# agis85/multimodal_segmentation

Hardware: AMD Instinct MI355X
Metric: 2D slices/sec DAFNet train step, 256x256x2-modality bs=8/GPU (higher is better)
Workload: dtype f32

## Files before the change

### include/mmseg_hip.h

```cpp
#ifndef MMSEG_HIP_H
#define MMSEG_HIP_H

#ifdef __cplusplus
extern "C" {
#endif

#define MMSEG_ACT_NONE 0
#define MMSEG_ACT_RELU 1
#define MMSEG_ACT_LEAKY 2
#define MMSEG_ACT_TANH 3

int mmseg_conv2d_fwd(const float* x1, const float* x2, const float* w, const float* wt, const float* bias, float* y, float* y2,
                     int B, int H, int W, int C1, int C2, int Ho, int Wo, int Cout, int KH, int KW, int stride,
                     int pad_h, int pad_w, int ups, int transposed, int act, float alpha, int nsplit1, void* stream);
int mmseg_set_conv_precision(int mode);
int mmseg_conv16_mode(int mode);
int mmseg_get_conv_precision(void);
int mmseg_conv2d_fwd_scaled(const float* x1, const float* x2, const float* w, const float* wt, const float* bias, const float* oscale,
                            float* y, int B, int H, int W, int C1, int C2, int Ho, int Wo, int Cout, int KH, int KW, int stride,
                            int pad_h, int pad_w, int ups, int act, float alpha, void* stream);
int mmseg_conv2d_fwd_t(const void* x1, const void* x2, const float* w, const float* wt, const float* bias, void* y, void* y2,
                       int B, int H, int W, int C1, int C2, int Ho, int Wo, int Cout, int KH, int KW, int stride,
                       int pad_h, int pad_w, int ups, int transposed, int act, float alpha, int nsplit1, int io, void* stream);
int mmseg_conv2d_fwd_scaled_t(const void* x1, const void* x2, const float* w, const float* wt, const float* bias, const float* oscale,
// ... 94 lines not shown
int mmseg_cat_words(const void* p0, const void* p1, const void* p2, const void* p3, const void* p4, const void* p5, const void* p6,
                    const void* p7, int n, void* out, long words, void* stream);
int mmseg_gather_rows(const void* src, const long long* idx, void* out, int rows, long words, int src_rows, void* stream);
int mmseg_add_residual(const float* msk, float* out, long M, int C, void* stream);
int mmseg_act_bwd_bias_t(const void* dy, const void* y, void* dx, float* bias_grad, float* ws, long M, int C, int act, float alpha,
                         int accumulate, int h, void* stream);
int mmseg_im2col8_t(const void* x, void* out, int B, int H, int W, int hx, int hy, void* stream);
int mmseg_conv8h_fwd_t(const void* x, const float* w, const float* bias, void* y, int B, int H, int W, int Cout, int act, float alpha,
                       int hx, int hy, void* stream);
int mmseg_in_workspace_floats(int B);
int mmseg_instnorm_spade_fwd(const float* x, const float* gamma, const float* beta, float* y, float* stat, float* ws, int B,
                             long per_sample, float eps, float act_alpha, void* stream);
int mmseg_instnorm_spade_bwd(const float* dy, const float* x, const float* stat, const float* gamma, const float* beta, float* dx,
                             float* dgamma, float* dbeta, float* dxn, float* ws, int B, long per_sample, float eps, float act_alpha,
                             void* stream);
int mmseg_instnorm_spade_fwd_gb(const float* x, const float* gb, float* y, float* stat, float* ws, int B, long per_sample, int C, float eps,
                                float act_alpha, void* stream);
int mmseg_instnorm_spade_bwd_gb(const float* dy, const float* x, const float* stat, const float* gb, float* dx, float* dgb, float* dxn,
                                float* ws, int B, long per_sample, int C, float eps, float act_alpha, void* stream);
int mmseg_instnorm_spade_fwd_gb_t(const float* x, const void* gb, void* y, float* stat, float* ws, int B, long per_sample, int C, float eps,
                                  float act_alpha, int h, int hy, void* stream);
int mmseg_instnorm_spade_bwd_gb_t(const void* dy, const float* x, const float* stat, const void* gb, float* dx, void* dgb, float* dxn,
                                  float* ws, int B, long per_sample, int C, float eps, float act_alpha, int h, int hy, void* stream);
int mmseg_colsum_t(const void* x, float* out, float* ws, long M, int C, int accumulate, int h, void* stream);
int mmseg_concat_cols(const float* a, const float* b, float* out, long M, int Ca, int Cb, void* stream);
int mmseg_split_cols_acc(const float* src, float* da, float* db, long M, int Ca, int Cb, void* stream);


long mmseg_dense_workspace_floats(int R, int K, int N);
int mmseg_dense_fwd(const float* x, const float* w, const float* bias, float* y, float* ws, int R, int K, int N, int act,
                    float alpha, void* stream);
int mmseg_dense_dgrad(const float* dy, const float* w, float* dx, int R, int K, int N, void* stream);
int mmseg_dense_wgrad(const float* x, const float* dy, float* dw, int R, int K, int N, int accumulate, void* stream);

int mmseg_tps_workspace_floats(int B);
int mmseg_tps_warp_fwd(const float* vol, const float* theta, const float* Mb, float* out, float* loc, int B, int H, int W, int C,
                       void* stream);
long mmseg_tps_scatter_workspace_floats(int B, int H, int W, int C);
int mmseg_tps_warp_bwd(const float* vol, const float* loc, const float* Mb, const float* dout, float* dvol, float* dtheta, float* dloc,
                       float* ws, float* acc, int B, int H, int W, int C, void* stream);

int mmseg_affine_gather(const float* data, const int* rows, const float* mat, float* out, int B, int H, int W, int C, int order,
                        void* stream);
long mmseg_augment_workspace_floats(int B, int H, int W, int C);
int mmseg_augment_gather(const float* data, const int* rows, const double* mat, const float* shift, float* out, float* ws, int N,
                         int B, int H, int W, int C, int order, int fill_mode, float cval, void* stream);

int mmseg_segloss_workspace_floats(int B);
int mmseg_segloss_stats_floats(int B);
int mmseg_segloss_coef_floats(int B, int C);
int mmseg_segloss_class_offset(int B);
int mmseg_segloss_stats(const float* pred, const float* target, float* stats, float* ws, int B, long HW, int C, int nm, void* stream);
int mmseg_segloss_finalize(const float* stats, float* loss, float* coef, int B, int C, float n_pix_global, float n_pix_grad,
                           float lambda_bce, void* stream);
int mmseg_segloss_grad(const float* pred, const float* target, const float* coef, float* dpred, int B, long HW, int C, int nm,
                       float scale, int use_bce, void* stream);
int mmseg_segloss_grad_s(const float* pred, const float* target, const float* coef, float* dpred, int B, long HW, int C, int nm,
                         float scale, const float* scale_dev, int use_bce, void* stream);
int mmseg_pairloss_workspace_floats(int B);
int mmseg_pair_dice_fwd(const float* a, const float* b, float* stats, float* out, int ldo, float* ws, int B, long per_sample,
                        void* stream);
int mmseg_pair_dice_bwd(const float* a, const float* b, const float* stats, const float* g, int ldg, float* da, float* db,
                        int accumulate_a, int B, long per_sample, void* stream);
int mmseg_row_mae_fwd(const float* x, const float* y, float* out, float* ws, int B, long per_sample, void* stream);
int mmseg_row_mae_bwd(const float* x, const float* y, const float* g, float* dy, int B, long per_sample, void* stream);
int mmseg_segpb_stats_floats(int B);
int mmseg_segpb_class_offset(int B);
int mmseg_segpb_stats(const float* pred, const float* target, float* stats, float* ws, int B, long HW, int C, int nm, void* stream);
int mmseg_segpb_loss(const float* stats, float* loss, int B, long HW, int C, float lambda_bce, void* stream);
int mmseg_segpb_classgrad(const float* stats, const float* g, float* A, int B, void* stream);
int mmseg_segpb_grad(const float* target, const float* stats, const float* g, const float* A, float* dpred, int B, long HW, int C,
                     int nm, float lambda_bce, void* stream);
int mmseg_rowdot_fwd(const float* w, const float* l, float* out, int B, int J, void* stream);
int mmseg_rowdot_bwd(const float* w, const float* l, const float* g, float* dw, float* dl, int B, int J, void* stream);

int mmseg_diffloss_workspace_floats(void);
int mmseg_diffloss(const float* p, const float* t, float tconst, long n, int mode, float* loss, float* ws, void* stream);
int mmseg_diffloss_grad(const float* p, const float* t, float tconst, long n, int mode, float scale, float* dp, void* stream);
int mmseg_diffloss_grad_s(const float* p, const float* t, float tconst, long n, int mode, float scale, const float* scale_dev, float* dp,
                          void* stream);

int mmseg_adam(float* p, const float* g, float* m, float* v, long n, float lr_t, float b1, float b2, float eps, void* stream);
int mmseg_adam_p(float* p, const float* g, float* m, float* v, long n, const float* lr_t, float b1, float b2, float eps, void* stream);
long mmseg_spectral_workspace_floats(int K, int N);
int mmseg_spectral_fwd(const float* w, const float* u0, float* loss, float* sgn, float* ws, int K, int N, float alpha, void* stream);
int mmseg_spectral_grad(const float* w, const float* sgn, float scale, long n, float* dw, void* stream);
int mmseg_spectral_fwd4(const float* w0, const float* w1, const float* w2, const float* w3, const float* u0, const float* u1,
                        const float* u2, const float* u3, float* loss, float* sgn, float* ws, int n, int K0, int N0, int K1, int N1,
                        int K2, int N2, int K3, int N3, float alpha, void* stream);
int mmseg_spectral_grad4(const float* w0, const float* w1, const float* w2, const float* w3, const float* sgn, float* dw0, float* dw1,
                         float* dw2, float* dw3, int n, long n0, long n1, long n2, long n3, float scale, void* stream);
int mmseg_spectral_grad4_s(const float* w0, const float* w1, const float* w2, const float* w3, const float* sgn, float* dw0, float* dw1,
                           float* dw2, float* dw3, int n, long n0, long n1, long n2, long n3, float scale, const float* scale_dev,
                           void* stream);

int mmseg_unscale_check8(float* g0, float* g1, float* g2, float* g3, float* g4, float* g5, float* g6, float* g7, long n0, long n1,
                         long n2, long n3, long n4, long n5, long n6, long n7, int count, const float* scale, int* st, void* stream);
int mmseg_adam_guarded(float* p, const float* g, float* m, float* v, long n, const float* lr_table, int table_len, const int* st,
                       float b1, float b2, float eps, void* stream);
int mmseg_loss_scale_update(float* scale, int* st, int growth_interval, void* stream);

long mmseg_preprocess_workspace_floats(int S, int RH, int RW);
int mmseg_preprocess_minmax(const float* img, float* ws, int S, int H, int W, int RH, int RW, void* stream);
int mmseg_preprocess_image(const float* img, const float* ws, float* out, int S, int H, int W, int RH, int RW, int OH, int OW, int lo_r,
                           int kept_r, int before_r, int lo_c, int kept_c, int before_c, int C, int ch, void* stream);
int mmseg_preprocess_label(const unsigned char* lab, const int* values, float* out, int S, int H, int W, int RH, int RW, int OH, int OW,
                           int lo_r, int kept_r, int before_r, int lo_c, int kept_c, int before_c, int C, int ch0, int K, void* stream);

int mmseg_restore_label(const float* prob, const int* values, unsigned char* out, int S, int H, int W, int RH, int RW, int OH, int OW,
                        int lo_r, int kept_r, int before_r, int lo_c, int kept_c, int before_c, int C, int K, int order, void* stream);
int mmseg_label_overlap(const unsigned char* pred, const unsigned char* truth, const int* values, int* counts, int S, int n, int K,
                        void* stream);

// ... 35 lines not shown
```

### multimodal_segmentation_amd/csrc/dense.hip

```cpp
#include "common.hpp"

#define DENSE_KSLICES_MAX 1024

static inline int dense_kslices(int K) {
    int ks = (K + 127) / 128;
    if (ks > DENSE_KSLICES_MAX) ks = DENSE_KSLICES_MAX;
    if (ks < 1) ks = 1;
    return ks;
}

template <int RB>
__global__ void dense_fwd_partial_kernel(const float* __restrict__ x, const float* __restrict__ w, float* __restrict__ part,
                                         int R, int K, int N, int kper) {
    __shared__ float red[4][RB][64];
    const int nl = threadIdx.x & 63, kl = threadIdx.x >> 6;
    const int n = blockIdx.x * 64 + nl;
    const int kbeg = blockIdx.y * kper, kend = min(K, kbeg + kper);
    float acc[RB];
#pragma unroll
    for (int b = 0; b < RB; ++b) acc[b] = 0.f;
    if (n < N) {
#pragma unroll 4
        for (int k = kbeg + kl; k < kend; k += 4) {
            const float wv = w[(size_t)k * N + n];
// ... 160 lines not shown
__global__ __launch_bounds__(256) void dense_dgrad_smallk_kernel(const float* __restrict__ dy, const float* __restrict__ w,
                                                                 float* __restrict__ dx, int K, int N) {
    __shared__ float red[17];
    const int b = blockIdx.x;
    float acc[KMAX];
#pragma unroll
    for (int k = 0; k < KMAX; ++k) acc[k] = 0.f;
    for (int n = threadIdx.x; n < N; n += 256) {
        const float d = dy[(size_t)b * N + n];
#pragma unroll
        for (int k = 0; k < KMAX; ++k)
            if (k < K) acc[k] = fmaf(d, w[(size_t)k * N + n], acc[k]);
    }
#pragma unroll
    for (int k = 0; k < KMAX; ++k) {
        if (k < K) {
            const float t = block_sum(acc[k], red);
            if (threadIdx.x == 0) dx[(size_t)b * K + k] = t;
        }
    }
}

__global__ void dense_wgrad_kernel(const float* __restrict__ x, const float* __restrict__ dy, float* __restrict__ dw,
                                   int R, int K, int N, int accumulate) {
    const long total = (long)K * N;
    for (long i = (long)blockIdx.x * blockDim.x + threadIdx.x; i < total; i += (long)gridDim.x * blockDim.x) {
        const int k = i / N, n = i - (long)k * N;
        float a = 0.f;
        for (int b = 0; b < R; ++b) a += x[(size_t)b * K + k] * dy[(size_t)b * N + n];
        dw[i] = accumulate ? dw[i] + a : a;
    }
}

extern "C" {

long mmseg_dense_workspace_floats(int R, int K, int N) {
    const long a = (long)dense_kslices(K) * R * N, b = (long)((K + SMALLN_KPB - 1) / SMALLN_KPB) * R * N;
    return a > b ? a : b;
}

int mmseg_dense_fwd(const float* x, const float* w, const float* bias, float* y, float* ws, int R, int K, int N, int act,
                    float alpha, void* stream) {
    if (R < 1 || R > 32) return (int)hipErrorInvalidValue;
    hipStream_t st = (hipStream_t)stream;
    if (N <= 4 && (R <= 16 || N == 1) && K >= 4096) {
        const int nb = (K + SMALLN_KPB - 1) / SMALLN_KPB;
        if (R > 16) {
            hipLaunchKernelGGL((dense_fwd_smalln_kernel<32, 1>), dim3(nb), dim3(256), 0, st, x, w, ws, R, K, N);
        } else if (R <= 8) {
            if (N == 1) hipLaunchKernelGGL((dense_fwd_smalln_kernel<8, 1>), dim3(nb), dim3(256), 0, st, x, w, ws, R, K, N);
            else hipLaunchKernelGGL((dense_fwd_smalln_kernel<8, 4>), dim3(nb), dim3(256), 0, st, x, w, ws, R, K, N);
        } else {
            if (N == 1) hipLaunchKernelGGL((dense_fwd_smalln_kernel<16, 1>), dim3(nb), dim3(256), 0, st, x, w, ws, R, K, N);
            else hipLaunchKernelGGL((dense_fwd_smalln_kernel<16, 4>), dim3(nb), dim3(256), 0, st, x, w, ws, R, K, N);
        }
        hipLaunchKernelGGL(dense_fwd_final_kernel, dim3((R * N + 63) / 64), dim3(256), 0, st, (const float*)ws, bias, y, R, N, nb, act, alpha);
        return MMSEG_CHECK_LAUNCH();
    }
    const int ks = dense_kslices(K);
    int kper = (K + ks - 1) / ks;
    dim3 grid((N + 63) / 64, ks), block(256);
    if (K % 4 == 0 && (reinterpret_cast<uintptr_t>(x) & 15) == 0) {
        kper = (kper + 3) / 4 * 4;
        if (R <= 8) hipLaunchKernelGGL(dense_fwd_partial_k4_kernel<8>, grid, block, 0, st, x, w, ws, R, K, N, kper);
        else if (R <= 16) hipLaunchKernelGGL(dense_fwd_partial_k4_kernel<16>, grid, block, 0, st, x, w, ws, R, K, N, kper);
        else hipLaunchKernelGGL(dense_fwd_partial_k4_kernel<32>, grid, block, 0, st, x, w, ws, R, K, N, kper);
        hipLaunchKernelGGL(dense_fwd_final_kernel, dim3((R * N + 63) / 64), dim3(256), 0, st, (const float*)ws, bias, y, R, N, ks, act, alpha);
// ... 27 lines not shown
```

### multimodal_segmentation_amd/csrc/loss.hip

```cpp
#include "common.hpp"

#define LOSS_CHUNKS 128
#define SEG_MAXC 8

__global__ void segloss_partial_kernel(const float* __restrict__ pred, const float* __restrict__ target, float* __restrict__ part,
                                       long HW, int C, int nm) {
    __shared__ float red[17];
    const int b = blockIdx.y;
    const long per = (HW + LOSS_CHUNKS - 1) / LOSS_CHUNKS;
    const long p0 = (long)blockIdx.x * per, p1 = min(HW, p0 + per);
    float sI = 0.f, sT = 0.f, sP = 0.f, n[SEG_MAXC], S[SEG_MAXC];
#pragma unroll
    for (int c = 0; c < SEG_MAXC; ++c) { n[c] = 0.f; S[c] = 0.f; }
    for (long px = p0 + threadIdx.x; px < p1; px += blockDim.x) {
        const size_t o = ((size_t)b * HW + px) * C;
#pragma unroll
        for (int c = 0; c < SEG_MAXC; ++c) {
            if (c < C) {
                const float p = pred[o + c], t = target[o + c];
                if (c < nm) { sI += t * p; sT += t; sP += p; }
                n[c] += p;
                S[c] += p * logf(t + 1e-12f);
            }
        }
// ... 108 lines not shown
    if (threadIdx.x == 0) part[blockIdx.x] = a;
}
__global__ void diffloss_final_kernel(const float* __restrict__ part, int nblk, float inv_n, float* __restrict__ loss) {
    __shared__ float red[17];
    float a = 0.f;
    for (int i = threadIdx.x; i < nblk; i += blockDim.x) a += part[i];
    a = block_sum(a, red);
    if (threadIdx.x == 0) loss[0] = a * inv_n;
}
__global__ void diffloss_grad_kernel(const float* __restrict__ p, const float* __restrict__ t, float tconst, long n, int mode,
                                     float scale, float* __restrict__ dp) {
    for (long i = (long)blockIdx.x * blockDim.x + threadIdx.x; i < n; i += (long)gridDim.x * blockDim.x) {
        const float d = p[i] - (t ? t[i] : tconst);
        float g;
        if (mode == 0) g = d > 0.f ? 1.f : (d < 0.f ? -1.f : 0.f);
        else if (mode == 1) g = 2.f * d;
        else g = 1.f;
        dp[i] = g * scale;
    }
}
__global__ void diffloss_grad_s_kernel(const float* __restrict__ p, const float* __restrict__ t, float tconst, long n, int mode,
                                       float scale_host, const float* __restrict__ scale_dev, float* __restrict__ dp) {
    const float scale = scale_host * scale_dev[0];
    for (long i = (long)blockIdx.x * blockDim.x + threadIdx.x; i < n; i += (long)gridDim.x * blockDim.x) {
        const float d = p[i] - (t ? t[i] : tconst);
        float g;
        if (mode == 0) g = d > 0.f ? 1.f : (d < 0.f ? -1.f : 0.f);
        else if (mode == 1) g = 2.f * d;
        else g = 1.f;
        dp[i] = g * scale;
    }
}

static inline int lgrid(long n) {
    long b = (n + 255) / 256;
    if (b > 1024) b = 1024;
    if (b < 1) b = 1;
    return (int)b;
}

extern "C" {

int mmseg_segloss_workspace_floats(int B) { return B * LOSS_CHUNKS * (3 + 2 * SEG_MAXC); }
int mmseg_segloss_stats_floats(int B) { return B * 3 + 2 * SEG_MAXC; }
int mmseg_segloss_coef_floats(int B, int C) { return 2 * B + 2 * C; }
int mmseg_segloss_class_offset(int B) { return 3 * B; }

int mmseg_segloss_stats(const float* pred, const float* target, float* stats, float* ws, int B, long HW, int C, int nm, void* stream) {
    if (C > SEG_MAXC || nm > C || B * 3 > 1024) return (int)hipErrorInvalidValue;
    hipStream_t st = (hipStream_t)stream;
    hipLaunchKernelGGL(segloss_partial_kernel, dim3(LOSS_CHUNKS, B), dim3(256), 0, st, pred, target, ws, HW, C, nm);
    hipLaunchKernelGGL(segloss_stats_final_kernel, dim3(1), dim3(1024), 0, st, (const float*)ws, stats, B);
    return MMSEG_CHECK_LAUNCH();
}
int mmseg_segloss_finalize(const float* stats, float* loss, float* coef, int B, int C, float n_pix_global, float n_pix_grad, float lambda_bce, void* stream) {
    hipLaunchKernelGGL(segloss_finalize_kernel, dim3(1), dim3(64), 0, (hipStream_t)stream, stats, loss, coef, B, C, n_pix_global, n_pix_grad, lambda_bce);
    return MMSEG_CHECK_LAUNCH();
}
int mmseg_segloss_grad(const float* pred, const float* target, const float* coef, float* dpred, int B, long HW, int C, int nm,
                       float scale, int use_bce, void* stream) {
    const long n = (long)B * HW * C;
    hipLaunchKernelGGL(segloss_grad_kernel, dim3(lgrid(n) * 4), dim3(256), 0, (hipStream_t)stream, pred, target, coef, dpred, B, HW, C, nm, scale, use_bce);
    return MMSEG_CHECK_LAUNCH();
}
int mmseg_segloss_grad_s(const float* pred, const float* target, const float* coef, float* dpred, int B, long HW, int C, int nm,
                         float scale, const float* scale_dev, int use_bce, void* stream) {
    if (scale_dev == nullptr) return (int)hipErrorInvalidValue;
    const long n = (long)B * HW * C;
    hipLaunchKernelGGL(segloss_grad_s_kernel, dim3(lgrid(n) * 4), dim3(256), 0, (hipStream_t)stream, pred, target, coef, dpred, B, HW, C,
                       nm, scale, scale_dev, use_bce);
    return MMSEG_CHECK_LAUNCH();
}

int mmseg_diffloss_workspace_floats(void) { return 1024; }
int mmseg_diffloss(const float* p, const float* t, float tconst, long n, int mode, float* loss, float* ws, void* stream) {
    hipStream_t st = (hipStream_t)stream;
    const int nblk = lgrid(n);
    hipLaunchKernelGGL(diffloss_partial_kernel, dim3(nblk), dim3(256), 0, st, p, t, tconst, n, mode, ws);
    hipLaunchKernelGGL(diffloss_final_kernel, dim3(1), dim3(256), 0, st, (const float*)ws, nblk, 1.f / (float)n, loss);
    return MMSEG_CHECK_LAUNCH();
}
int mmseg_diffloss_grad(const float* p, const float* t, float tconst, long n, int mode, float scale, float* dp, void* stream) {
    hipLaunchKernelGGL(diffloss_grad_kernel, dim3(lgrid(n) * 4), dim3(256), 0, (hipStream_t)stream, p, t, tconst, n, mode, scale, dp);
    return MMSEG_CHECK_LAUNCH();
}
int mmseg_diffloss_grad_s(const float* p, const float* t, float tconst, long n, int mode, float scale, const float* scale_dev, float* dp,
                          void* stream) {
    if (scale_dev == nullptr) return (int)hipErrorInvalidValue;
    hipLaunchKernelGGL(diffloss_grad_s_kernel, dim3(lgrid(n) * 4), dim3(256), 0, (hipStream_t)stream, p, t, tconst, n, mode, scale, scale_dev,
                       dp);
    return MMSEG_CHECK_LAUNCH();
}

}
```

### multimodal_segmentation_amd/model_components/decoder.py

```python
import logging

from .. import nn, ops
from ..layers import spade
from ..utils.rng import global_rng

log = logging.getLogger('decoder')


class Decoder(nn.Model):
    def __init__(self, conf, rng):
        super(Decoder, self).__init__('Decoder')
        self.conf = conf
        self.decoder_type = conf.decoder_type
        sc = conf.anatomy_encoder.output_shape[-1]
        if conf.decoder_type == 'film':
            nn.conv_params(self, 'c0', 3, sc, 8)
            for i in range(4):
                nn.conv_params(self, 'f%d_c1' % i, 3, 8, 8)
                nn.conv_params(self, 'f%d_c2' % i, 3, 8, 8)
                nn.dense_params(self, 'f%d_gamma' % i, conf.num_z, 8)
                nn.dense_params(self, 'f%d_beta' % i, conf.num_z, 8)
            last = 8
        elif conf.decoder_type == 'spade':
            last = spade.declare_spade_decoder(self, conf)
        else:
            raise ValueError('Unknown decoder_type value: ' + str(conf.decoder_type))
        nn.conv_params(self, 'out', 1, last, 1, 'glorot_normal')
        self.finalize(rng)
        self.output_shape = (None,) + tuple(conf.input_shape)

    def _film_decoder(self, s, z):
        l = nn.conv(self, 'c0', s, act='leaky', alpha=0.3)
        zs = ops.Shared(z, 8)
        for i in range(4):
            n = 'f%d' % i
            l1 = ops.Shared(nn.conv(self, n + '_c1', l, act='leaky', alpha=0.3), 2)
            l2 = nn.conv(self, n + '_c2', l1.use())
            gamma = nn.dense(self, n + '_gamma', zs.use(), act='leaky', alpha=0.3)
            beta = nn.dense(self, n + '_beta', zs.use(), act='leaky', alpha=0.3)
            l = ops.film(l2, gamma, beta, res=l1.use(), alpha=0.3)
        return l

    def forward(self, s, z, training=False):
        if self.decoder_type == 'film':
            l = self._film_decoder(s, z)
        else:
            l = spade.spade_decoder(self, self.conf, s, z)
        return nn.conv(self, 'out', l, act='tanh')


def build(conf, rng=None):
    model = Decoder(conf, rng or global_rng())
    log.info('Decoder')
    model.summary(print_fn=log.debug)
    return model
```

### multimodal_segmentation_amd/models/trainer.py

```python
import torch

from .. import graphs, nn, ops
from ..parallel import dp


class OutputSpec(object):
    __slots__ = ('name', 'kind', 'weight')

    def __init__(self, name, kind, weight):
        self.name, self.kind, self.weight = name, kind, float(weight)


class Trainer(object):
    def __init__(self, name, graph_fn, output_specs, train_models, optimizer, num_masks=None, regularised=(),
                 all_models=()):
        self.name = name
        self.graph_fn = graph_fn
        self.specs = list(output_specs)
        self.train_models = list(train_models)
        self.optimizer = optimizer
        self.num_masks = num_masks
        self.regularised = list(regularised)
        self.all_models = list(all_models) or self.train_models
        self.device = self.train_models[0].device
        self.last_outputs = None
        self.use_graph = False
        self._graphs = {}
        self.loss_scale = 1.0
        self.scaler = None
        self.precision = None

    @property
    def output_names(self):
        return [s.name for s in self.specs]

    def summary(self, print_fn=print):
        print_fn('Trainer %s: %d outputs, trainable models: %s' % (self.name, len(self.specs),
                                                                   ', '.join(m.name for m in self.train_models)))

    def _loss_and_grad(self, spec, pred, target):
        gs = spec.weight * self.loss_scale
        sd = self.scaler.scale_dev if self.scaler is not None else None
        if spec.kind == 'dice_bce':
            return ops.seg_loss(pred, target, self.num_masks, 0.01, gs, class_sum_hook=dp.class_sum_hook(),
                                n_pix_global=pred.numel() // pred.shape[-1] * dp.world_size(), scale_dev=sd)
        if spec.kind == 'dice':
            return ops.seg_loss(pred, target, self.num_masks, 0.0, gs, scale_dev=sd)
        if spec.kind == 'mse':
            return ops.diff_loss(pred, target, 'mse', gs, scale_dev=sd)
        if spec.kind == 'mae':
            return ops.diff_loss(pred, target, 'mae', gs, scale_dev=sd)
        if spec.kind == 'ypred':
            return ops.diff_loss(pred, 0.0, 'mean', gs, scale_dev=sd)
        raise ValueError(spec.kind)

    def _prep_target(self, t, pred):
        if isinstance(t, (int, float)):
            return float(t)
        t = nn.to_device(t, self.device)
        if t.numel() != pred.numel():
            t = t.reshape(-1, *([1] * (pred.dim() - 1))).expand_as(pred).contiguous()
        return t

    def fit(self, inputs, targets, epochs=1, verbose=0, **graph_kw):
        assert epochs == 1
        inputs = list(inputs) if isinstance(inputs, (list, tuple)) else [inputs]
        targets = list(targets) if isinstance(targets, (list, tuple)) else [targets]
        graph_kw = {k: v for k, v in graph_kw.items() if v is not None}
        with ops.precision_scope(self.precision):
            if self.use_graph and not graph_kw and not dp.enabled() and self.device.type == 'cuda':
                key = graphs.signature(inputs, targets)
                st = self._graphs.get(key)
                if st is None:
                    st = self._graphs[key] = graphs.FitGraph(self)
                return st.run(inputs, targets)
            return self._fit_eager(inputs, targets, graph_kw)

    @staticmethod
    def _total(terms):
        return nn_total(terms)

    def _fit_eager(self, inputs, targets, graph_kw, lr_dev=None):
        ins = [nn.to_device(x, self.device) for x in inputs]
        assert len(targets) == len(self.specs), '%s: %d targets for %d outputs' % (self.name, len(targets), len(self.specs))
        for m in self.train_models:
            m.zero_grad_own()
        tracker = dp.begin(self.train_models, defer=[d for d in self.regularised if d in self.train_models])
        with torch.enable_grad():
            outs = self.graph_fn(ins, **graph_kw)
            assert len(outs) == len(self.specs)
            hist = nn.History()
            grads, terms = [], []
            for spec, pred, tgt in zip(self.specs, outs, targets):
                loss, dpred = self._loss_and_grad(spec, pred, self._prep_target(tgt, pred))
                grads.append(dpred)
                terms.append((spec.weight, loss))
                hist.record(spec.name + '_loss', loss)
            torch.autograd.backward(outs, grads)
        for d in self.regularised:
            kw = {} if self.scaler is None else {'grad_scale_dev': self.scaler.scale_dev}
            for loss in d.regulariser_losses(accumulate_grad=d in self.train_models, grad_scale=self.loss_scale, **kw):
                terms.append((1.0, loss))
        dp.finish(tracker)
        if self.scaler is not None:
            self.scaler.unscale_(self.train_models)
            self.scaler.step(self.train_models)
        else:
            if self.loss_scale != 1.0:
                for m in self.train_models:
                    ops.axpby(m.grad_arena, m.grad_arena, 1.0 / self.loss_scale, 0.0, out=m.grad_arena)
            self.optimizer.step(self.train_models, lr_dev=lr_dev)
        hist.record('loss', nn_total(terms))
        self.last_outputs = [o.detach() for o in outs]
        return hist

    def predict(self, inputs, **graph_kw):
        ins = [nn.to_device(x, self.device) for x in (inputs if isinstance(inputs, (list, tuple)) else [inputs])]
        with torch.no_grad(), ops.precision_scope(self.precision):
            outs = self.graph_fn(ins, training=False, **graph_kw)
        return [nn.to_numpy(o) for o in outs]


class nn_total(object):

    def __init__(self, terms):
        self.terms = terms

# ... 3 lines not shown
```

### multimodal_segmentation_amd/nn.py

```python
import itertools
import math
import weakref
from collections import OrderedDict

import numpy as np
import torch

from . import ops
from .parallel import dp

_DEVICE = None


def default_device():
    global _DEVICE
    if _DEVICE is None:
        if torch.cuda.is_available():
            _DEVICE = torch.device('cuda', torch.cuda.current_device())
        else:
            _DEVICE = torch.device('cpu')
    return _DEVICE


def set_default_device(dev):
# ... 257 lines not shown
def dense_params(m, name, cin, cout, init='glorot_uniform'):
    m.add_param(name + '/kernel', (cin, cout), init)
    m.add_param(name + '/bias', (cout,), 'zeros')


def bn_params(m, name, c):
    m.add_param(name + '/gamma', (c,), 'ones')
    m.add_param(name + '/beta', (c,), 'zeros')
    m.add_param(name + '/moving_mean', (c,), 'zeros', trainable=False)
    m.add_param(name + '/moving_variance', (c,), 'ones', trainable=False)


def conv(m, name, x, stride=1, padding='same', act=None, alpha=0.0, x2=None, upsample=False, bias_grad=True, out_dtype=torch.float32):
    w = m.params[name + '/kernel']
    b = m.params.get(name + '/bias')
    return ops.conv2d(x, w.data, b.data if b is not None else None, stride, padding, act, alpha, x2, upsample,
                      wgrad=w.g(), bgrad=b.g() if (b is not None and bias_grad) else None, anchor=anchor(x.device),
                      wkey=(w.uid, w.owner.uid), out_dtype=out_dtype)


def conv_pair(m, name_a, name_b, x, out_dtype=torch.float32):
    wa, ba = m.params[name_a + '/kernel'], m.params[name_a + '/bias']
    wb, bb = m.params[name_b + '/kernel'], m.params[name_b + '/bias']
    grads = (wa.g(), ba.g(), wb.g(), bb.g())
    return ops.conv2d_pair(x, wa.data, ba.data, wb.data, bb.data, grads, anchor=anchor(x.device), wkey=(wa.uid, wa.owner.uid),
                           out_dtype=out_dtype)


def dense(m, name, x, act=None, alpha=0.0):
    w, b = m.params[name + '/kernel'], m.params[name + '/bias']
    return ops.dense(x, w.data, b.data, act, alpha, wgrad=w.g(), bgrad=b.g(), anchor=anchor(x.device))


def bn(m, name, x, training, relu=False, out_dtype=torch.float32):
    g, b = m.params[name + '/gamma'], m.params[name + '/beta']
    return ops.batchnorm(x, g.data, b.data, m.params[name + '/moving_mean'].data,
                         m.params[name + '/moving_variance'].data, training, relu,
                         ggrad=g.g(), bgrad=b.g(), anchor=anchor(x.device), out_dtype=out_dtype)


def conv_bn(m, cname, bname, x, training, relu=False, x2=None, upsample=False, y16=True):
    w, b = m.params[cname + '/kernel'], m.params.get(cname + '/bias')
    half = ops.act16_dtype()
    Cout = w.shape[3]
    c1 = x.shape[3]
    c2 = x2.shape[3] if x2 is not None else 0
    conv_dt = half if (half is not None and c1 % 32 == 0 and c2 % 32 == 0 and Cout % 64 == 0) else torch.float32
    bn_dt = half if (half is not None and y16 and Cout % 64 == 0) else torch.float32
    if training or torch.is_grad_enabled():
        l = conv(m, cname, x, x2=x2, upsample=upsample, bias_grad=not training, out_dtype=conv_dt)
        return bn(m, bname, l, training, relu=relu, out_dtype=bn_dt)
    return ops.conv2d_bn_infer(x, w.data, b.data if b is not None else None, m.params[bname + '/gamma'].data,
                               m.params[bname + '/beta'].data, m.params[bname + '/moving_mean'].data,
                               m.params[bname + '/moving_variance'].data, relu=relu, x2=x2, upsample=upsample, wkey=(w.uid, w.owner.uid),
                               out_dtype=bn_dt)


def norm_params(m, name, c, norm):
    if norm == 'batch':
        bn_params(m, name, c)
    elif norm == 'instance':
        m.add_param(name + '/gamma', (1,), 'ones')
        m.add_param(name + '/beta', (1,), 'zeros')


def conv_norm(m, cname, nname, x, training, relu=False, x2=None, upsample=False, norm='batch'):
# ... 74 lines not shown
```

### multimodal_segmentation_amd/ops.py

```python
import torch

from . import _native as N
from .parallel import dp

ACT = {None: 0, 'linear': 0, 'relu': 1, 'leaky': 2, 'tanh': 3}
BN_EPS = 1e-3
BN_MOMENTUM = 0.99
IN_EPS = 1e-3

_workspaces = {}


def _sid(device):
    if device.type != 'cuda':
        return 0
    from . import graphs
    st = graphs._recording
    if st is not None and st.mode == 'capture':
        return ('graph', st.uid)
    return torch.cuda.current_stream(device).cuda_stream


def _ws(tag, n, device, dtype=torch.float32):
    key = (tag, device, _sid(device))
    buf = _workspaces.get(key)
    n = max(int(n), 1)
    if buf is None or buf.numel() < n:
        buf = torch.empty(max(n, 1024), dtype=dtype, device=device)
        _workspaces[key] = buf
    return buf


def _new(shape, like, dtype=torch.float32):
    return torch.empty(shape, dtype=dtype, device=like.device)


_act16 = [None]
_HCODE = {torch.float32: 0, torch.bfloat16: 1, torch.float16: 2}


def set_activation_storage(on):
    old = _act16[0]
    if not on:
        _act16[0] = None
        return old is not None
    mode = N.call('mmseg_get_conv_precision')
    if mode == 0:
        raise ValueError("16-bit activation storage needs compute_dtype 'bf16' or 'fp16'")
    _act16[0] = torch.bfloat16 if mode == 1 else torch.float16
    return old is not None


def act16_dtype():
    return _act16[0]


def _h(t):
    return 0 if t is None else _HCODE[t.dtype]


def _c(t):
    return t if t.is_contiguous() else t.contiguous()


_PRECISIONS = ['fp32', 'bf16', 'fp16']


# ... 717 lines not shown
        x, y = ctx.saved_tensors
        w = ctx.w
        R, K = x.shape
        Nn = w.shape[1]
        dy = _c(dy)
        if ctx.act:
            g = _new(dy.shape, dy)
            N.call('mmseg_act_bwd', dy, y, g, dy.numel(), ctx.act, float(ctx.alpha))
        else:
            g = dy
        dx = None
        if ctx.needs_input_grad[0]:
            dx = _new(x.shape, x)
            for r0 in range(0, R, _DENSE_ROWS):
                r = min(_DENSE_ROWS, R - r0)
                N.call('mmseg_dense_dgrad', g[r0:r0 + r], w, dx[r0:r0 + r], r, K, Nn)
        if ctx.wgrad is not None:
            for r0 in range(0, R, _DENSE_ROWS):
                r = min(_DENSE_ROWS, R - r0)
                N.call('mmseg_dense_wgrad', x[r0:r0 + r], g[r0:r0 + r], ctx.wgrad.view(-1), r, K, Nn, 1)
        if ctx.bgrad is not None:
            ws = _ws('colsum', N.call('mmseg_colsum_workspace_floats', R, Nn), x.device)
            N.call('mmseg_colsum', g, ctx.bgrad, ws, R, Nn, 1.0, 1)
        _grad_done(ctx.wgrad, ctx.bgrad)
        return (dx,) + (None,) * 7


def dense(x, w, bias=None, act=None, alpha=0.0, wgrad=None, bgrad=None, anchor=None):
    if wgrad is None and bgrad is None:
        anchor = None
    return _Dense.apply(x, anchor, w, bias, act, alpha, wgrad, bgrad)


class _Film(torch.autograd.Function):
    @staticmethod
    def forward(ctx, x, gamma, beta, res, alpha):
        x, gamma, beta = _c(x), _c(gamma), _c(beta)
        B, H, W, C = x.shape
        assert gamma.shape == (B, C) and beta.shape == (B, C)
        y = _new(x.shape, x)
        N.call('mmseg_film_fwd', x, gamma, beta, _c(res) if res is not None else None, y, B, H * W, C, float(alpha))
        ctx.alpha, ctx.has_res = alpha, res is not None
        ctx.save_for_backward(x, gamma, beta)
        return y

    @staticmethod
    def backward(ctx, dy):
        x, gamma, beta = ctx.saved_tensors
        B, H, W, C = x.shape
        dy = _c(dy)
        dx = _new(x.shape, x)
        dg, db = _new((B, C), x), _new((B, C), x)
        ws = _ws('film', N.call('mmseg_film_bwd_workspace', B, C), x.device)
        N.call('mmseg_film_bwd', dy, x, gamma, beta, dx, dg, db, ws, B, H * W, C, float(ctx.alpha))
        return dx, dg, db, (dy if ctx.has_res else None), None


def film(x, gamma, beta, res=None, alpha=0.3):
    return _Film.apply(x, gamma, beta, res, alpha)


class _TpsWarp(torch.autograd.Function):
    @staticmethod
    def forward(ctx, vol, theta, Mb):
        vol, theta = _c(vol), _c(theta)
        B, H, W, C = vol.shape
# ... 448 lines not shown
        B, J = w.shape
        dw, dl = _new(w.shape, w), _new(l.shape, l)
        N.call('mmseg_rowdot_bwd', w, l, _c(g), dw, dl, B, J)
        return (dw,) + tuple(dl[:, j].reshape(shp) for j, shp in enumerate(ctx.shapes))


def row_dot(w, ls):
    return _RowDot.apply(w, *ls)


_DIFF_MODE = {'mae': 0, 'mse': 1, 'mean': 2}


def diff_loss(pred, target, mode, scale, want_grad=True, scale_dev=None):
    pred = _c(pred)
    n = pred.numel()
    t, tc = (None, float(target)) if not isinstance(target, torch.Tensor) else (_c(target), 0.0)
    if t is not None:
        assert t.numel() == n
    loss = _new((1,), pred)
    ws = _ws('diffloss', N.call('mmseg_diffloss_workspace_floats'), pred.device)
    N.call('mmseg_diffloss', pred, t, tc, n, _DIFF_MODE[mode], loss, ws)
    dpred = None
    if want_grad:
        dpred = _new(pred.shape, pred)
        g = {0: 1.0 / n, 1: 1.0 / n, 2: 1.0 / n}[_DIFF_MODE[mode]] * scale
        if scale_dev is None:
            N.call('mmseg_diffloss_grad', pred, t, tc, n, _DIFF_MODE[mode], float(g), dpred)
        else:
            N.call('mmseg_diffloss_grad_s', pred, t, tc, n, _DIFF_MODE[mode], float(g), scale_dev, dpred)
    return loss, dpred


def spectral_reg(w, u0, alpha=10.0):
    K = w.numel() // w.shape[-1]
    Nn = w.shape[-1]
    assert u0.numel() == K
    loss, sgn = _new((1,), w), _new((1,), w)
    ws = _ws('spectral', N.call('mmseg_spectral_workspace_floats', K, Nn), w.device)
    N.call('mmseg_spectral_fwd', w, u0, loss, sgn, ws, K, Nn, float(alpha))
    return loss, sgn


def spectral_reg_multi(ws_, u0s, alpha=10.0):
    n = len(ws_)
    assert 1 <= n <= 4 and len(u0s) == n
    dims = [(w.numel() // w.shape[-1], w.shape[-1]) for w in ws_]
    loss, sgn = _new((n,), ws_[0]), _new((n,), ws_[0])
    need = sum(N.call('mmseg_spectral_workspace_floats', K, Nn) for K, Nn in dims)
    ws = _ws('spectral', need, ws_[0].device)
    pad = lambda lst, fill: list(lst) + [fill] * (4 - n)
    flat = [v for d in pad(dims, dims[0]) for v in d]
    N.call('mmseg_spectral_fwd4', *pad(ws_, ws_[0]), *pad(u0s, u0s[0]), loss, sgn, ws, n, *flat, float(alpha))
    return loss, sgn


def spectral_reg_grad_accumulate(ws_, sgn, grads, scale=1.0, scale_dev=None):
    n = len(ws_)
    pad = lambda lst, fill: list(lst) + [fill] * (4 - n)
    if scale_dev is None:
        N.call('mmseg_spectral_grad4', *pad(ws_, ws_[0]), sgn, *pad(grads, grads[0]), n, *pad([w.numel() for w in ws_], 0), float(scale))
    else:
        N.call('mmseg_spectral_grad4_s', *pad(ws_, ws_[0]), sgn, *pad(grads, grads[0]), n, *pad([w.numel() for w in ws_], 0),
               float(scale), scale_dev)


# ... 423 lines not shown
```

Baseline: 64.59.

## Batch FiLM dense layers and diff losses into grouped kernel launches

Adds grouped dense forward, dgrad and wgrad kernels that read pointer tables, so the decoder's eight FiLM gamma/beta dense layers run as one launch per pass instead of eight. Also adds a multi-term diff loss kernel that computes every mse/mae/ypred loss term and its gradient in a few launches. Both target kernel-launch and Python dispatch overhead from many tiny ops in the train step. In exchange it adds host-side ctypes table building, plain scalar (non-tiled) kernels, and a single shared gradient buffer for the loss terms.

```diff
diff --git a/include/mmseg_hip.h b/include/mmseg_hip.h
--- a/include/mmseg_hip.h
+++ b/include/mmseg_hip.h
@@ -150,6 +150,10 @@
                     float alpha, void* stream);
 int mmseg_dense_dgrad(const float* dy, const float* w, float* dx, int R, int K, int N, void* stream);
 int mmseg_dense_wgrad(const float* x, const float* dy, float* dw, int R, int K, int N, int accumulate, void* stream);
+int mmseg_dense_group_supported(int R, int K, int N);
+int mmseg_dense_group_fwd(const float* x, const long long* rows, int G, int R, int K, int N, int act, float alpha, void* stream);
+int mmseg_dense_group_dgrad(const long long* rows, float* dx, int G, int R, int K, int N, void* stream);
+int mmseg_dense_group_wgrad(const float* x, const long long* rows, int G, int R, int K, int N, int accumulate, void* stream);
 
 int mmseg_tps_workspace_floats(int B);
 int mmseg_tps_warp_fwd(const float* vol, const float* theta, const float* Mb, float* out, float* loc, int B, int H, int W, int C,
@@ -197,6 +201,10 @@
 int mmseg_diffloss_grad(const float* p, const float* t, float tconst, long n, int mode, float scale, float* dp, void* stream);
 int mmseg_diffloss_grad_s(const float* p, const float* t, float tconst, long n, int mode, float scale, const float* scale_dev, float* dp,
                           void* stream);
+long mmseg_diffloss_multi_workspace_floats(int nterms);
+int mmseg_diffloss_multi(const long long* rows, const float* frows, int nterms, float* loss, float* ws, void* stream);
+int mmseg_diffloss_grad_multi(const long long* rows, const float* frows, int nterms, float* dp, void* stream);
+int mmseg_diffloss_grad_multi_s(const long long* rows, const float* frows, int nterms, const float* scale_dev, float* dp, void* stream);
 
 int mmseg_adam(float* p, const float* g, float* m, float* v, long n, float lr_t, float b1, float b2, float eps, void* stream);
 int mmseg_adam_p(float* p, const float* g, float* m, float* v, long n, const float* lr_t, float b1, float b2, float eps, void* stream);
diff --git a/multimodal_segmentation_amd/csrc/dense.hip b/multimodal_segmentation_amd/csrc/dense.hip
--- a/multimodal_segmentation_amd/csrc/dense.hip
+++ b/multimodal_segmentation_amd/csrc/dense.hip
@@ -216,7 +216,147 @@
     }
 }
 
+#define DENSE_GROUP_MAX 16
+struct DenseGroupEnt { const float* w; const float* bias; const float* dy; float* out; };
+struct DenseGroupTable { DenseGroupEnt e[DENSE_GROUP_MAX]; };
+
+template <bool K4>
+__global__ __launch_bounds__(256) void dense_group_fwd_kernel(const float* __restrict__ x, const DenseGroupTable tb, int R, int K, int N,
+                                                              int act, float alpha) {
+    __shared__ float red[4][8][64];
+    const DenseGroupEnt& e = tb.e[blockIdx.z];
+    const float* __restrict__ w = e.w;
+    const int nl = threadIdx.x & 63, kl = threadIdx.x >> 6;
+    const int n = blockIdx.x * 64 + nl, b0 = blockIdx.y * 8;
+    float acc[8];
+#pragma unroll
+    for (int b = 0; b < 8; ++b) acc[b] = 0.f;
+    if (n < N) {
+        if (K4) {
+            for (int k = 4 * kl; k < K; k += 16) {
+                float wv[4];
+#pragma unroll
+                for (int q = 0; q < 4; ++q) wv[q] = w[(size_t)(k + q) * N + n];
+#pragma unroll
+                for (int b = 0; b < 8; ++b)
+                    if (b0 + b < R) {
+                        const f32x4 xv = *reinterpret_cast<const f32x4*>(x + (size_t)(b0 + b) * K + k);
+                        acc[b] += xv[0] * wv[0]; acc[b] += xv[1] * wv[1]; acc[b] += xv[2] * wv[2]; acc[b] += xv[3] * wv[3];
+                    }
+            }
+        } else {
+            for (int k = kl; k < K; k += 4) {
+                const float wv = w[(size_t)k * N + n];
+#pragma unroll
+                for (int b = 0; b < 8; ++b)
+                    if (b0 + b < R) acc[b] += x[(size_t)(b0 + b) * K + k] * wv;
+            }
+        }
+    }
+#pragma unroll
+    for (int b = 0; b < 8; ++b) red[kl][b][nl] = acc[b];
+    __syncthreads();
+    if (kl == 0 && n < N) {
+#pragma unroll
+        for (int b = 0; b < 8; ++b)
+            if (b0 + b < R) {
+                const float part = red[0][b][nl] + red[1][b][nl] + red[2][b][nl] + red[3][b][nl];
+                float t = 0.f;
+                t += part;
+                if (e.bias) t += e.bias[n];
+                e.out[(size_t)(b0 + b) * N + n] = act_apply(t, act, alpha);
+            }
+    }
+}
+
+__global__ __launch_bounds__(256) void dense_group_dgrad_kernel(const DenseGroupTable tb, int R, int K, int N) {
+    const DenseGroupEnt& e = tb.e[blockIdx.y];
+    const int i = blockIdx.x * 256 + threadIdx.x;
+    if (i >= R * K) return;
+    const int b = i / K, k = i - b * K;
+    const float* __restrict__ d = e.dy + (size_t)b * N;
+    const float* __restrict__ wr = e.w + (size_t)k * N;
+    float acc = 0.f;
+    for (int nb = 0; nb < N; nb += 128) {
+        const int nw = min(128, N - nb);
+        float a = 0.f;
+        for (int nn = 0; nn < nw; ++nn) a += d[nb + nn] * wr[nb + nn];
+        acc += a;
+    }
+    e.out[i] = acc;
+}
+
+__global__ __launch_bounds__(256) void dense_group_wgrad_kernel(const float* __restrict__ x, const DenseGroupTable tb, int R, int K, int N,
+                                                                int accumulate) {
+    const DenseGroupEnt& e = tb.e[blockIdx.y];
+    const int i = blockIdx.x * 256 + threadIdx.x;
+    if (i >= K * N) return;
+    const int k = i / N, n = i - k * N;
+    const float* __restrict__ dy = e.dy;
+    float v = accumulate ? e.out[i] : 0.f;
+    for (int r0 = 0; r0 < R; r0 += 32) {
+        const int r1 = min(R, r0 + 32);
+        float a = 0.f;
+        for (int b = r0; b < r1; ++b) a += x[(size_t)b * K + k] * dy[(size_t)b * N + n];
+        v = (accumulate || r0) ? v + a : a;
+    }
+    e.out[i] = v;
+}
+
+static int dense_group_table(DenseGroupTable& tb, const long long* rows, int first, int G, bool need_w, bool need_dy,
+                             float* stacked = nullptr, size_t per = 0) {
+    const int g = G - first < DENSE_GROUP_MAX ? G - first : DENSE_GROUP_MAX;
+    for (int k = 0; k < g; ++k) {
+        const long long* r = rows + (size_t)(first + k) * 4;
+        tb.e[k].w = reinterpret_cast<const float*>(r[0]);
+        tb.e[k].bias = reinterpret_cast<const float*>(r[1]);
+        tb.e[k].dy = reinterpret_cast<const float*>(r[2]);
+        tb.e[k].out = stacked ? stacked + (size_t)(first + k) * per : reinterpret_cast<float*>(r[3]);
+        if (tb.e[k].out == nullptr || (need_w && tb.e[k].w == nullptr) || (need_dy && tb.e[k].dy == nullptr)) return -1;
+    }
+    return g;
+}
+
 extern "C" {
+
+int mmseg_dense_group_supported(int R, int K, int N) {
+    return R >= 1 && K >= 1 && N >= 1 && K <= 128 && (long)R * K < (1L << 30) && (long)R * N < (1L << 30) && (long)K * N < (1L << 30) &&
+           (R + 7) / 8 <= 65535 &&
+           !(K <= 16 && N >= 1024) && !(N <= 4 && K >= 4096);
+}
+int mmseg_dense_group_fwd(const float* x, const long long* rows, int G, int R, int K, int N, int act, float alpha, void* stream) {
+    if (x == nullptr || rows == nullptr || G < 1 || !mmseg_dense_group_supported(R, K, N)) return (int)hipErrorInvalidValue;
+    const bool k4 = K % 4 == 0 && (reinterpret_cast<uintptr_t>(x) & 15) == 0;
+    DenseGroupTable tb;
+    for (int first = 0; first < G; first += DENSE_GROUP_MAX) {
+        const int g = dense_group_table(tb, rows, first, G, true, false);
+        if (g < 0) return (int)hipErrorInvalidValue;
+        const dim3 grid((N + 63) / 64, (R + 7) / 8, g);
+        if (k4) hipLaunchKernelGGL(dense_group_fwd_kernel<true>, grid, dim3(256), 0, (hipStream_t)stream, x, tb, R, K, N, act, alpha);
+        else hipLaunchKernelGGL(dense_group_fwd_kernel<false>, grid, dim3(256), 0, (hipStream_t)stream, x, tb, R, K, N, act, alpha);
+    }
+    return MMSEG_CHECK_LAUNCH();
+}
+int mmseg_dense_group_dgrad(const long long* rows, float* dx, int G, int R, int K, int N, void* stream) {
+    if (rows == nullptr || dx == nullptr || G < 1 || !mmseg_dense_group_supported(R, K, N)) return (int)hipErrorInvalidValue;
+    DenseGroupTable tb;
+    for (int first = 0; first < G; first += DENSE_GROUP_MAX) {
+        const int g = dense_group_table(tb, rows, first, G, true, true, dx, (size_t)R * K);
+        if (g < 0) return (int)hipErrorInvalidValue;
+        hipLaunchKernelGGL(dense_group_dgrad_kernel, dim3((R * K + 255) / 256, g), dim3(256), 0, (hipStream_t)stream, tb, R, K, N);
+    }
+    return MMSEG_CHECK_LAUNCH();
+}
+int mmseg_dense_group_wgrad(const float* x, const long long* rows, int G, int R, int K, int N, int accumulate, void* stream) {
+    if (x == nullptr || rows == nullptr || G < 1 || !mmseg_dense_group_supported(R, K, N)) return (int)hipErrorInvalidValue;
+    DenseGroupTable tb;
+    for (int first = 0; first < G; first += DENSE_GROUP_MAX) {
+        const int g = dense_group_table(tb, rows, first, G, false, true);
+        if (g < 0) return (int)hipErrorInvalidValue;
+        hipLaunchKernelGGL(dense_group_wgrad_kernel, dim3((K * N + 255) / 256, g), dim3(256), 0, (hipStream_t)stream, x, tb, R, K, N, accumulate);
+    }
+    return MMSEG_CHECK_LAUNCH();
+}
 
 long mmseg_dense_workspace_floats(int R, int K, int N) {
     const long a = (long)dense_kslices(K) * R * N, b = (long)((K + SMALLN_KPB - 1) / SMALLN_KPB) * R * N;
diff --git a/multimodal_segmentation_amd/csrc/loss.hip b/multimodal_segmentation_amd/csrc/loss.hip
--- a/multimodal_segmentation_amd/csrc/loss.hip
+++ b/multimodal_segmentation_amd/csrc/loss.hip
@@ -164,11 +164,94 @@
     }
 }
 
+#define DIFF_MULTI_MAX 32
+struct DiffTerm {
+    const float* p; const float* t; float* dp;
+    long n;
+    float tconst, inv_n, scale;
+    int mode, slot;
+    int blk0, nblk;
+    int gblk0;
+};
+struct DiffTable { DiffTerm e[DIFF_MULTI_MAX]; int nterms; };
+
+__device__ __forceinline__ int diff_term_of_block(const DiffTable& tb, int b, bool grad) {
+    int k = 0;
+    while (k + 1 < tb.nterms && (grad ? tb.e[k + 1].gblk0 : tb.e[k + 1].blk0) <= b) ++k;
+    return k;
+}
+__global__ void diffloss_multi_partial_kernel(const DiffTable tb, float* __restrict__ part) {
+    __shared__ float red[17];
+    const DiffTerm& e = tb.e[diff_term_of_block(tb, blockIdx.x, false)];
+    const float* __restrict__ p = e.p;
+    const float* __restrict__ t = e.t;
+    const float tconst = e.tconst;
+    const long n = e.n;
+    const int mode = e.mode, lb = blockIdx.x - e.blk0, nblk = e.nblk;
+    float a = 0.f;
+    for (long i = (long)lb * blockDim.x + threadIdx.x; i < n; i += (long)nblk * blockDim.x) {
+        const float d = p[i] - (t ? t[i] : tconst);
+        a += mode == 0 ? fabsf(d) : (mode == 1 ? d * d : p[i]);
+    }
+    a = block_sum(a, red);
+    if (threadIdx.x == 0) part[blockIdx.x] = a;
+}
+__global__ void diffloss_multi_final_kernel(const DiffTable tb, const float* __restrict__ part, float* __restrict__ loss) {
+    __shared__ float red[17];
+    const DiffTerm& e = tb.e[blockIdx.x];
+    const float* __restrict__ mine = part + e.blk0;
+    const int nblk = e.nblk;
+    float a = 0.f;
+    for (int i = threadIdx.x; i < nblk; i += blockDim.x) a += mine[i];
+    a = block_sum(a, red);
+    if (threadIdx.x == 0) loss[e.slot] = a * e.inv_n;
+}
+__global__ void diffloss_multi_grad_kernel(const DiffTable tb, const float* __restrict__ scale_dev) {
+    const DiffTerm& e = tb.e[diff_term_of_block(tb, blockIdx.x, true)];
+    const float* __restrict__ p = e.p;
+    const float* __restrict__ t = e.t;
+    float* __restrict__ dp = e.dp;
+    const float tconst = e.tconst, scale = scale_dev ? e.scale * scale_dev[0] : e.scale;
+    const long n = e.n;
+    const int mode = e.mode, lb = blockIdx.x - e.gblk0, nblk = 4 * e.nblk;
+    for (long i = (long)lb * blockDim.x + threadIdx.x; i < n; i += (long)nblk * blockDim.x) {
+        const float d = p[i] - (t ? t[i] : tconst);
+        float g;
+        if (mode == 0) g = d > 0.f ? 1.f : (d < 0.f ? -1.f : 0.f);
+        else if (mode == 1) g = 2.f * d;
+        else g = 1.f;
+        dp[i] = g * scale;
+    }
+}
+
 static inline int lgrid(long n) {
     long b = (n + 255) / 256;
     if (b > 1024) b = 1024;
     if (b < 1) b = 1;
     return (int)b;
+}
+
+static int diff_table(DiffTable& tb, const long long* rows, const float* frows, float* dp, int first, int nterms, int& blocks,
+                      int& gblocks) {
+    blocks = gblocks = 0;
+    tb.nterms = nterms - first < DIFF_MULTI_MAX ? nterms - first : DIFF_MULTI_MAX;
+    for (int k = 0; k < tb.nterms; ++k) {
+        const long long* r = rows + (size_t)(first + k) * 6;
+        DiffTerm& e = tb.e[k];
+        e.p = reinterpret_cast<const float*>(r[0]);
+        e.t = reinterpret_cast<const float*>(r[1]);
+        e.dp = dp ? dp + r[2] : nullptr;
+        e.n = (long)r[3];
+        e.mode = (int)r[4];
+        e.slot = (int)r[5];
+        if (e.p == nullptr || e.n < 1 || e.mode < 0 || e.mode > 2 || e.slot < 0 || (dp && r[2] < 0)) return (int)hipErrorInvalidValue;
+        e.tconst = frows[(size_t)(first + k) * 2];
+        e.scale = frows[(size_t)(first + k) * 2 + 1];
+        e.inv_n = 1.f / (float)e.n;
+        e.blk0 = blocks; e.nblk = lgrid(e.n); e.gblk0 = gblocks;
+        blocks += e.nblk; gblocks += 4 * e.nblk;
+    }
+    return 0;
 }
 
 extern "C" {
@@ -224,4 +307,36 @@
     return MMSEG_CHECK_LAUNCH();
 }
 
-}
+long mmseg_diffloss_multi_workspace_floats(int nterms) { return 1024L * (nterms < 1 ? 1 : nterms); }
+int mmseg_diffloss_multi(const long long* rows, const float* frows, int nterms, float* loss, float* ws, void* stream) {
+    if (rows == nullptr || frows == nullptr || nterms < 1) return (int)hipErrorInvalidValue;
+    hipStream_t st = (hipStream_t)stream;
+    DiffTable tb;
+    for (int first = 0; first < nterms; first += DIFF_MULTI_MAX) {
+        int blocks, gblocks;
+        if (const int rc = diff_table(tb, rows, frows, nullptr, first, nterms, blocks, gblocks)) return rc;
+        float* part = ws + (size_t)first * 1024;
+        hipLaunchKernelGGL(diffloss_multi_partial_kernel, dim3(blocks), dim3(256), 0, st, tb, part);
+        hipLaunchKernelGGL(diffloss_multi_final_kernel, dim3(tb.nterms), dim3(256), 0, st, tb, (const float*)part, loss);
+    }
+    return MMSEG_CHECK_LAUNCH();
+}
+static int diffloss_grad_multi(const long long* rows, const float* frows, int nterms, const float* scale_dev, float* dp, hipStream_t st) {
+    if (rows == nullptr || frows == nullptr || dp == nullptr || nterms < 1) return (int)hipErrorInvalidValue;
+    DiffTable tb;
+    for (int first = 0; first < nterms; first += DIFF_MULTI_MAX) {
+        int blocks, gblocks;
+        if (const int rc = diff_table(tb, rows, frows, dp, first, nterms, blocks, gblocks)) return rc;
+        hipLaunchKernelGGL(diffloss_multi_grad_kernel, dim3(gblocks), dim3(256), 0, st, tb, scale_dev);
+    }
+    return MMSEG_CHECK_LAUNCH();
+}
+int mmseg_diffloss_grad_multi(const long long* rows, const float* frows, int nterms, float* dp, void* stream) {
+    return diffloss_grad_multi(rows, frows, nterms, nullptr, dp, (hipStream_t)stream);
+}
+int mmseg_diffloss_grad_multi_s(const long long* rows, const float* frows, int nterms, const float* scale_dev, float* dp, void* stream) {
+    if (scale_dev == nullptr) return (int)hipErrorInvalidValue;
+    return diffloss_grad_multi(rows, frows, nterms, scale_dev, dp, (hipStream_t)stream);
+}
+
+}
diff --git a/multimodal_segmentation_amd/model_components/decoder.py b/multimodal_segmentation_amd/model_components/decoder.py
--- a/multimodal_segmentation_amd/model_components/decoder.py
+++ b/multimodal_segmentation_amd/model_components/decoder.py
@@ -32,12 +32,13 @@
     def _film_decoder(self, s, z):
         l = nn.conv(self, 'c0', s, act='leaky', alpha=0.3)
         zs = ops.Shared(z, 8)
+        names = ['f%d_%s' % (i, p) for i in range(4) for p in ('gamma', 'beta')]
+        gb = nn.dense_group(self, names, [zs.use() for _ in names], act='leaky', alpha=0.3)
         for i in range(4):
             n = 'f%d' % i
             l1 = ops.Shared(nn.conv(self, n + '_c1', l, act='leaky', alpha=0.3), 2)
             l2 = nn.conv(self, n + '_c2', l1.use())
-            gamma = nn.dense(self, n + '_gamma', zs.use(), act='leaky', alpha=0.3)
-            beta = nn.dense(self, n + '_beta', zs.use(), act='leaky', alpha=0.3)
+            gamma, beta = gb[2 * i], gb[2 * i + 1]
             l = ops.film(l2, gamma, beta, res=l1.use(), alpha=0.3)
         return l
 
diff --git a/multimodal_segmentation_amd/models/trainer.py b/multimodal_segmentation_amd/models/trainer.py
--- a/multimodal_segmentation_amd/models/trainer.py
+++ b/multimodal_segmentation_amd/models/trainer.py
@@ -2,6 +2,9 @@
 
 from .. import graphs, nn, ops
 from ..parallel import dp
+
+
+_DIFF_KINDS = {'mse': 'mse', 'mae': 'mae', 'ypred': 'mean'}
 
 
 class OutputSpec(object):
@@ -46,13 +49,21 @@
                                 n_pix_global=pred.numel() // pred.shape[-1] * dp.world_size(), scale_dev=sd)
         if spec.kind == 'dice':
             return ops.seg_loss(pred, target, self.num_masks, 0.0, gs, scale_dev=sd)
-        if spec.kind == 'mse':
-            return ops.diff_loss(pred, target, 'mse', gs, scale_dev=sd)
-        if spec.kind == 'mae':
-            return ops.diff_loss(pred, target, 'mae', gs, scale_dev=sd)
-        if spec.kind == 'ypred':
-            return ops.diff_loss(pred, 0.0, 'mean', gs, scale_dev=sd)
         raise ValueError(spec.kind)
+
+    def _losses_and_grads(self, outs, targets):
+        targets = [self._prep_target(tgt, pred) for pred, tgt in zip(outs, targets)]
+        res = [None] * len(self.specs)
+        diff = [i for i, spec in enumerate(self.specs) if spec.kind in _DIFF_KINDS]
+        sd = self.scaler.scale_dev if self.scaler is not None else None
+        items = [(outs[i], 0.0 if self.specs[i].kind == 'ypred' else targets[i], _DIFF_KINDS[self.specs[i].kind],
+                  self.specs[i].weight * self.loss_scale) for i in diff]
+        for i, r in zip(diff, ops.diff_loss_multi(items, scale_dev=sd)):
+            res[i] = r
+        for i, spec in enumerate(self.specs):
+            if res[i] is None:
+                res[i] = self._loss_and_grad(spec, outs[i], targets[i])
+        return res
 
     def _prep_target(self, t, pred):
         if isinstance(t, (int, float)):
@@ -91,8 +102,7 @@
             assert len(outs) == len(self.specs)
             hist = nn.History()
             grads, terms = [], []
-            for spec, pred, tgt in zip(self.specs, outs, targets):
-                loss, dpred = self._loss_and_grad(spec, pred, self._prep_target(tgt, pred))
+            for spec, (loss, dpred) in zip(self.specs, self._losses_and_grads(outs, targets)):
                 grads.append(dpred)
                 terms.append((spec.weight, loss))
                 hist.record(spec.name + '_loss', loss)
diff --git a/multimodal_segmentation_amd/nn.py b/multimodal_segmentation_amd/nn.py
--- a/multimodal_segmentation_amd/nn.py
+++ b/multimodal_segmentation_amd/nn.py
@@ -313,6 +313,13 @@
     return ops.dense(x, w.data, b.data, act, alpha, wgrad=w.g(), bgrad=b.g(), anchor=anchor(x.device))
 
 
+def dense_group(m, names, xs, act=None, alpha=0.0):
+    ws = [m.params[n + '/kernel'] for n in names]
+    bs = [m.params[n + '/bias'] for n in names]
+    return ops.dense_group(xs, [w.data for w in ws], [b.data for b in bs], act, alpha, wgrads=[w.g() for w in ws],
+                           bgrads=[b.g() for b in bs], anchor=anchor(xs[0].device))
+
+
 def bn(m, name, x, training, relu=False, out_dtype=torch.float32):
     g, b = m.params[name + '/gamma'], m.params[name + '/beta']
     return ops.batchnorm(x, g.data, b.data, m.params[name + '/moving_mean'].data,
diff --git a/multimodal_segmentation_amd/ops.py b/multimodal_segmentation_amd/ops.py
--- a/multimodal_segmentation_amd/ops.py
+++ b/multimodal_segmentation_amd/ops.py
@@ -1,3 +1,5 @@
+import ctypes
+
 import torch
 
 from . import _native as N
@@ -33,6 +35,36 @@
 
 def _new(shape, like, dtype=torch.float32):
     return torch.empty(shape, dtype=dtype, device=like.device)
+
+
+_batched = [True]
+
+
+def set_batched_launches(on):
+    old = _batched[0]
+    _batched[0] = bool(on)
+    return old
+
+
+class _HostTable(object):
+
+    def __init__(self, rows, frows=None):
+        flat = [int(v) for r in rows for v in r]
+        self._rows = (ctypes.c_longlong * len(flat))(*flat)
+        self.rows = ctypes.addressof(self._rows)
+        if frows is not None:
+            flat = [float(v) for r in frows for v in r]
+            self._frows = (ctypes.c_float * len(flat))(*flat)
+            self.frows = ctypes.addressof(self._frows)
+
+
+def _addr(t, like):
+    if t is None:
+        return 0
+    if t.dtype != torch.float32 or not t.is_contiguous() or t.device != like.device:
+        raise ValueError('kernel operand must be a contiguous fp32 tensor on %s (got %s %s contiguous=%s)'
+                         % (like.device, t.dtype, t.device, t.is_contiguous()))
+    return t.data_ptr()
 
 
 _act16 = [None]
@@ -816,6 +848,69 @@
     return _Dense.apply(x, anchor, w, bias, act, alpha, wgrad, bgrad)
 
 
+class _DenseGroup(torch.autograd.Function):
+
+    @staticmethod
+    def forward(ctx, anchor, ws_, biases, act, alpha, wgrads, bgrads, *xs):
+        assert all(a.data_ptr() == xs[0].data_ptr() and a.shape == xs[0].shape and a.stride() == xs[0].stride() for a in xs)
+        x = _c(xs[0])
+        R, K = x.shape
+        Nn = ws_[0].shape[1]
+        ys = [_new((R, Nn), x) for _ in ws_]
+        tb = _HostTable([(_addr(w, x), _addr(b, x), 0, y.data_ptr()) for w, b, y in zip(ws_, biases, ys)])
+        N.call('mmseg_dense_group_fwd', x, tb.rows, len(ws_), R, K, Nn, ACT[act], float(alpha))
+        ctx.act, ctx.alpha = ACT[act], alpha
+        ctx.ws, ctx.wgrads, ctx.bgrads = ws_, wgrads, bgrads
+        ctx.save_for_backward(x, *(ys if ACT[act] else ()))
+        return tuple(ys)
+
+    @staticmethod
+    def backward(ctx, *dys):
+        x, ys = ctx.saved_tensors[0], ctx.saved_tensors[1:]
+        R, K = x.shape
+        G, Nn = len(ctx.ws), ctx.ws[0].shape[1]
+        gs = []
+        for i, dy in enumerate(dys):
+            dy = _c(dy)
+            if ctx.act:
+                g = _new(dy.shape, dy)
+                N.call('mmseg_act_bwd', dy, ys[i], g, dy.numel(), ctx.act, float(ctx.alpha))
+            else:
+                g = dy
+            gs.append(g)
+        dxs = [None] * G
+        if any(ctx.needs_input_grad[7:]):
+            dx = _new((G, R, K), x)
+            tb = _HostTable([(_addr(w, x), 0, _addr(g, x), 0) for w, g in zip(ctx.ws, gs)])
+            N.call('mmseg_dense_group_dgrad', tb.rows, dx, G, R, K, Nn)
+            dxs = list(dx.unbind(0))
+        if ctx.wgrads[0] is not None:
+            tb = _HostTable([(0, 0, _addr(g, x), _addr(dw, x)) for g, dw in zip(gs, ctx.wgrads)])
+            N.call('mmseg_dense_group_wgrad', x, tb.rows, G, R, K, Nn, 1)
+        for g, bgrad in zip(gs, ctx.bgrads):
+            if bgrad is not None:
+                ws = _ws('colsum', N.call('mmseg_colsum_workspace_floats', R, Nn), x.device)
+                N.call('mmseg_colsum', g, bgrad, ws, R, Nn, 1.0, 1)
+        _grad_done(*(list(ctx.wgrads) + list(ctx.bgrads)))
+        return (None,) * 7 + tuple(dxs)
+
+
+def dense_group(xs, ws_, biases, act=None, alpha=0.0, wgrads=None, bgrads=None, anchor=None):
+    G = len(ws_)
+    wgrads = list(wgrads) if wgrads is not None else [None] * G
+    bgrads = list(bgrads) if bgrads is not None else [None] * G
+    x = xs[0]
+    grouped = (_batched[0] and x.is_cuda and x.dim() == 2 and len(xs) == G and all(w.shape == ws_[0].shape for w in ws_)
+               and len(set(g is None for g in wgrads)) == 1
+               and N.call('mmseg_dense_group_supported', x.shape[0], x.shape[1], ws_[0].shape[1]))
+    if not grouped:
+        return [dense(xs[i], ws_[i], biases[i], act, alpha, wgrads[i], bgrads[i], anchor) for i in range(G)]
+    assert x.shape[1] == ws_[0].shape[0], 'dense: input has %d features, kernel expects %d' % (x.shape[1], ws_[0].shape[0])
+    if all(g is None for g in wgrads + bgrads):
+        anchor = None
+    return list(_DenseGroup.apply(anchor, list(ws_), list(biases), act, alpha, wgrads, bgrads, *xs))
+
+
 class _Film(torch.autograd.Function):
     @staticmethod
     def forward(ctx, x, gamma, beta, res, alpha):
@@ -1330,6 +1425,36 @@
     return loss, dpred
 
 
+def diff_loss_multi(items, want_grad=True, scale_dev=None):
+    if len(items) < 2 or not _batched[0] or not items[0][0].is_cuda:
+        return [diff_loss(pred, target, mode, scale, want_grad, scale_dev) for pred, target, mode, scale in items]
+    first = items[0][0]
+    losses = _new((len(items),), first)
+    keep, rows, frows, off = [], [], [], 0
+    for k, (pred, target, mode, scale) in enumerate(items):
+        pred = _c(pred)
+        n = pred.numel()
+        t, tc = (None, float(target)) if not isinstance(target, torch.Tensor) else (_c(target), 0.0)
+        if t is not None:
+            assert t.numel() == n
+        keep.append((pred, t))
+        rows.append((_addr(pred, first), _addr(t, first), off, n, _DIFF_MODE[mode], k))
+        frows.append((tc, 1.0 / n * scale))
+        off += (n + 3) // 4 * 4
+    tb = _HostTable(rows, frows)
+    ws = _ws('diffloss_multi', N.call('mmseg_diffloss_multi_workspace_floats', len(items)), first.device)
+    N.call('mmseg_diffloss_multi', tb.rows, tb.frows, len(items), losses, ws)
+    dpreds = [None] * len(items)
+    if want_grad:
+        dp_all = _new((off,), first)
+        if scale_dev is None:
+            N.call('mmseg_diffloss_grad_multi', tb.rows, tb.frows, len(items), dp_all)
+        else:
+            N.call('mmseg_diffloss_grad_multi_s', tb.rows, tb.frows, len(items), scale_dev, dp_all)
+        dpreds = [dp_all[r[2]:r[2] + r[3]].view(pred.shape) for r, (pred, _) in zip(rows, keep)]
+    return [(losses[k:k + 1], dpreds[k]) for k in range(len(items))]
+
+
 def spectral_reg(w, u0, alpha=10.0):
     K = w.numel() // w.shape[-1]
     Nn = w.shape[-1]
```

Measured after the change: 64.86, median of 6. No clear change (+0.4%).
